# NeSC-IV/sage-icp

Hardware: AMD Instinct MI355X
Metric: ICP frames/sec (120k-pt scan vs 1M-pt map) (higher is better)
Workload: dtype f64

## Files before the change

sage-icp_amd/csrc/icp_body.h:

```cpp
#pragma once

namespace sageicp {

#ifndef SAGE_LOOP_FLAT_MINW
#define SAGE_LOOP_FLAT_MINW 8
#endif
#ifndef SAGE_SCAN_AHEAD
#define SAGE_SCAN_AHEAD 1
#endif
#ifndef SAGE_ROW_SHIFT_LAYER
#define SAGE_ROW_SHIFT_LAYER 1
#endif
#ifndef SAGE_ROW_SHIFT_MAXW
#define SAGE_ROW_SHIFT_MAXW 4
#endif

struct PairCompact {
    uint4 a, b;
    unsigned ka, oa;
    bool ha, hb;
};
struct PairFull {
    Point4 a, b;
    unsigned ka;
// ... 9 lines not shown
    unsigned ka, kb;
    bool ha, hb;
};

__device__ __forceinline__ unsigned icp_wave_of_stripe(const IcpParams &P, int wv, unsigned &stripe_id) {
    constexpr unsigned kStripe = SAGE_ICP_STRIPE;
    const unsigned xcd = blockIdx.x & 7u, jb = blockIdx.x >> 3;
    unsigned stripe = (jb / kStripe) * 8u + xcd;
    if (P.stripe_order) {
        const unsigned nstripes = gridDim.x / kStripe;
        switch (stripe * 4u / nstripes) {
            case 0: __builtin_amdgcn_s_setprio(3); break;
            case 1: __builtin_amdgcn_s_setprio(2); break;
            case 2: __builtin_amdgcn_s_setprio(1); break;
            default: break;
        }
        stripe = P.stripe_order[stripe];
    }
    stripe_id = stripe;
    const unsigned wg = stripe * kStripe + (jb % kStripe);
    return wg * static_cast<unsigned>(kIcpWavesPerBlock) + static_cast<unsigned>(wv);
}

__device__ __forceinline__ void axis_gaps(double v, int k, double vs, double sc, double (&g)[3]) {
    const double below_hi = static_cast<double>(k <= 0 ? k - 1 : k) * vs;
    const double above_lo = static_cast<double>(k >= 0 ? k + 1 : k) * vs;
    const double slack = 1e-9 * vs + 1e-13 * fabs(v);
    const double lo = fmax((v - below_hi) - slack, 0.0);
    const double hi = fmax((above_lo - v) - slack, 0.0);
    g[0] = (lo * lo) * sc;
    g[1] = 0.0;
    g[2] = (hi * hi) * sc;
}

__device__ __forceinline__ float round_up_f32(double x) {
    return __uint_as_float(__float_as_uint(static_cast<float>(x)) + 1u);
}

template <int LW>
__device__ __forceinline__ bool reduce_argmin(double best, unsigned bkey, bool valid, const uint32_t *lrow, unsigned &mkey, unsigned &woff) {
    constexpr int W = 1 << LW, SH = 5;
    const double m = seg_min_f64<W>(best);
    const unsigned mine = (best == m) ? bkey : 0xFFFFFFFFu;
    mkey = seg_min_u32<W>(mine);
    const bool found = valid && mkey != 0xFFFFFFFFu;
    woff = (lrow[found ? mkey >> 8 : 0u] >> 8) * (kUnitPoints * 32u) + ((mkey & 255u) << SH);
    return found;
}

template <int LW, bool FUSED, bool FILT, bool PERSIST = false, bool FLATQ = false>
// ... 76 lines not shown
        f = P.frame[qc];
        auto row_piece = [&](int k) {
            const unsigned p = min(ci + static_cast<unsigned>(W * k), 6u);
            return *reinterpret_cast<const uint4 *>(grow + 4u * p);
        };
        pc0 = row_piece(0); pc1 = pc0; pc2 = pc0; pc3 = pc0; pc4 = pc0; pc5 = pc0; pc6 = pc0;
        if (NP > 1) pc1 = row_piece(1);
        if (NP > 2) pc2 = row_piece(2);
        if (NP > 3) pc3 = row_piece(3);
        if (NP > 4) pc4 = row_piece(4);
        if (NP > 5) pc5 = row_piece(5);
        if (NP > 6) pc6 = row_piece(6);
    }
    PROBE_DELAY_WAIT(P, t0);
    if constexpr (FUSED && !PERSIST) {
        if (P.chain && P.chain_iter > 0) {
            if (wv == 0) chain_wait_pose(P, smem, lane);
            __syncthreads();
            if (smem[kWgGo]) return;
        }
    }
    const Query s = [&]() {
        if constexpr (PERSIST) {
            return make_query<(W >= 4)>(f, pose, pose + 9, 1, P.voxel_size, P.inv_voxel_size);
        } else if constexpr (FUSED) {
            const double *lpose = reinterpret_cast<const double *>(smem + kWgPose);
            return make_query<(W >= 4)>(f, lpose, lpose + 9, P.apply_pose, P.voxel_size, P.inv_voxel_size);
        } else {
            return make_query<(W >= 4)>(f, P.st->R, P.st->T + 4, P.apply_pose, P.voxel_size, P.inv_voxel_size);
        }
    }();
    const bool stale = valid && (static_cast<uint32_t>(s.kx) != rk.x || static_cast<uint32_t>(s.ky) != rk.y ||
                                 static_cast<uint32_t>(s.kz) != rk.z);
    unsigned occ = rk.w;
    NN_T(np, 0);
    LP_T(PERSIST, G, 0);
    if constexpr (!PERSIST) {
        auto stage = [&](int k, const uint4 &v) {
            const unsigned p = ci + static_cast<unsigned>(W * k);
            if (p < 7u) *reinterpret_cast<uint4 *>(lrow + 4u * p) = v;
        };
        stage(0, pc0);
        if (NP > 1) stage(1, pc1);
        if (NP > 2) stage(2, pc2);
        if (NP > 3) stage(3, pc3);
        if (NP > 4) stage(4, pc4);
        if (NP > 5) stage(5, pc5);
        if (NP > 6) stage(6, pc6);
    }
    if (__ballot(stale)) {
        if (stale) {
            unsigned o = 0u, cq = 0u;
// ... 123 lines not shown
                    start(v2, s2, e2);
                    finish(v0, s0, e0);
                    finish(v1, s1, e1);
                    finish(v2, s2, e2);
                }
            }
            o = seg_or_u32<W>(o);
            cq = seg_add_u32<W>(cq);
            occ = o;
            if (ci == 0u) {
                lrow[kRowCq] = cq;
                if constexpr (!PERSIST) {
                    uint4 t;
                    t.x = static_cast<uint32_t>(s.kx); t.y = static_cast<uint32_t>(s.ky);
                    t.z = static_cast<uint32_t>(s.kz); t.w = o;
                    *reinterpret_cast<uint4 *>(P.rows + static_cast<size_t>(q) * kRowWords + kRowKey) = t;
                    P.rows[static_cast<size_t>(q) * kRowWords + kRowCq] = cq;
                }
            }
            if constexpr (PERSIST) {
                if (ci == 0u) {
                    *reinterpret_cast<uint2 *>(lst + kStKey) = make_uint2(static_cast<uint32_t>(s.kx), static_cast<uint32_t>(s.ky));
                    *reinterpret_cast<uint2 *>(lst + kStKey + 2) = make_uint2(static_cast<uint32_t>(s.kz), o);
                }
            }
        }
    }
    if (!valid) occ = 0u;

    double gx[3], gy[3], gz[3];
    {
        const double vs = P.voxel_size, sc = P.prune_scale;
        axis_gaps(s.x, s.kx, vs, sc, gx);
        axis_gaps(s.y, s.ky, vs, sc, gy);
        axis_gaps(s.z, s.kz, vs, sc, gz);
    }
    NN_T(np, 1);
    LP_T(PERSIST, G, 1);

    double best = P.dist_init;
    unsigned bkey = 0xFFFFFFFFu;
    const int pli = static_cast<int>(s.l);
    const double th = P.sem_th;
    unsigned npairs = 0u;

    unsigned k = ci, kend = 0u, off = 0u;
    unsigned pk = 0u, needs = 0u, wn = 0u;
    auto evaluate = [&](const Point4 &nb, bool on, unsigned key) {
        const double dx = nb.x - s.x, dy = nb.y - s.y, dz = nb.z - s.z;
        double d = SAGE_SQNORM3_NN(dx * dx, dy * dy, dz * dz);
        const bool same = static_cast<int>(nb.l) == pli || fabs(nb.l * s.l) < 1.0;
        const double ds = d * th;
        d = same ? ds : d;
        d = __hiloint2double(on ? __double2hiint(d) : 0x7FF80000, __double2loint(d));
        const bool lt = d < best, eq = d == best, kl = key < bkey;
        const bool take = lt | (eq & kl);
        best = min_f64(best, d);
        bkey = take ? key : bkey;
// ... 213 lines not shown
            for (int c = 0; c < 3; ++c) {
                const double lb = ga + (gy[b] + gz[c]);
                layer |= (lb <= bound) ? (1u << (3 * b + c)) : 0u;
            }
        }
        layer = (a < 3u && ci < 4u) ? layer << (9u * a) : 0u;
        layer |= dpp_u32<kDppXor1>(layer);
        layer |= dpp_u32<kDppXor2>(layer);
        if (W >= 8) layer |= dpp_u32<kDppHalfMirror>(layer);
        if (W >= 16) layer |= dpp_u32<kDppMirror>(layer);
        need |= layer & ~(1u << kHome);
    } else {
#pragma unroll
        for (int v = 0; v < 27; ++v) {
            if (v == static_cast<int>(kHome)) continue;
            const double lb = gx[v / 9] + (gy[(v / 3) % 3] + gz[v % 3]);
            need |= (lb <= bound) ? (1u << v) : 0u;
        }
    }
    LP_T(PERSIST, G, 3);
    scan((merged ? (need | (1u << kHome)) : (need & ~(1u << kHome))) & occ, nullptr, false, 0u);
    LP_T(PERSIST, G, 4);
    if constexpr (PERSIST) {
        if (valid && ci == 0u)
            (void)__hip_atomic_fetch_max(G->work + bslot, npairs + (stale ? 48u : 0u), __ATOMIC_RELAXED, __HIP_MEMORY_SCOPE_WORKGROUP);
    }

    unsigned mkey, woff;
    const bool found = reduce_argmin<LW>(best, bkey, valid, lrow, mkey, woff);
    NN_T(np, 3);
    LP_T(PERSIST, G, 5);

    if (P.counters) {
        const unsigned long long ab = (valid && ci == 0u)
                                          ? (static_cast<unsigned long long>(lrow[kRowCq]) << 32) | npairs : 0ull;
        unsigned lo = static_cast<unsigned>(ab), hi = static_cast<unsigned>(ab >> 32);
        lo += dpp_u32<kDppXor1>(lo);        hi += dpp_u32<kDppXor1>(hi);
        lo += dpp_u32<kDppXor2>(lo);        hi += dpp_u32<kDppXor2>(hi);
        lo += dpp_u32<kDppHalfMirror>(lo);  hi += dpp_u32<kDppHalfMirror>(hi);
        lo += dpp_u32<kDppMirror>(lo);      hi += dpp_u32<kDppMirror>(hi);
        unsigned b = 0u, a = 0u;
#pragma unroll
        for (int r = 0; r < 4; ++r) {
            b += static_cast<unsigned>(__builtin_amdgcn_readlane(static_cast<int>(lo), 16 * r));
            a += static_cast<unsigned>(__builtin_amdgcn_readlane(static_cast<int>(hi), 16 * r));
        }
        if (lane == 0 && wave_id < P.nwaves) {
            (void)__hip_atomic_fetch_add(&P.counters[2u * wave_id], static_cast<unsigned long long>(a),
                                         __ATOMIC_RELAXED, __HIP_MEMORY_SCOPE_AGENT);
            (void)__hip_atomic_fetch_add(&P.counters[2u * wave_id + 1u], static_cast<unsigned long long>(b),
                                         __ATOMIC_RELAXED, __HIP_MEMORY_SCOPE_AGENT);
        }
    }

    if (!FUSED) {
        if (valid && ci == 0u) P.nn_idx[q] = found ? static_cast<int>(woff >> SH) : -1;
    } else {
        if constexpr (!PERSIST) {
            if (valid && ci == 0u) P.nn_prev[q] = make_uint2(found ? mkey : 0xFFFFFFFFu, woff);
        }
        Point4 g;
        if constexpr (PERSIST) {
            const bool changed = found && mkey != prev.x;
            g = *reinterpret_cast<const Point4 *>(lst + 8);
            if (__ballot(changed)) {
                const Point4 t = load_point(pts, changed ? woff : 0u);
                if (changed) {
                    g = t;
                    if (ci == 0u) *reinterpret_cast<Point4 *>(lst + 8) = t;
                }
            }
            if (ci == 0u) *reinterpret_cast<uint2 *>(lst + kStPrev) = make_uint2(found ? mkey : 0xFFFFFFFFu, woff);
            LP_T(PERSIST, G, 6);
        }
        PROBE_NN_WORK(P, q, valid && ci == 0u, npairs);
        constexpr int K = kCount >> LW;
        double t[K];
        if constexpr (!PERSIST) g = load_point(pts, found ? woff : 0u);
        const double rx0 = s.x - g.x, ry0 = s.y - g.y, rz0 = s.z - g.z;
        const bool use = found && SAGE_SQNORM3_ACCEPT(rx0 * rx0, ry0 * ry0, rz0 * rz0) <= P.accept_r2;
        {
            const double r2 = SAGE_SQNORM3_RESID(rx0 * rx0, ry0 * ry0, rz0 * rz0);
            const double k = P.kernel;
            const double den = k + r2;
            const double wq = (k * k) / (den * den);
            const bool z = W == 1;
            const double w = !z || use ? wq : 0.0;
            const double sx = !z || use ? s.x : 0.0, sy = !z || use ? s.y : 0.0, sz = !z || use ? s.z : 0.0;
            const double rx = !z || use ? rx0 : 0.0, ry = !z || use ? ry0 : 0.0, rz = !z || use ? rz0 : 0.0;
            const double wsx = w * sx, wsy = w * sy, wsz = w * sz;
            double u[kCount];
            u[kW] = w;
            u[kWsx] = wsx; u[kWsy] = wsy; u[kWsz] = wsz;
            u[kWxx] = wsx * sx; u[kWxy] = wsx * sy; u[kWxz] = wsx * sz;
            u[kWyy] = wsy * sy; u[kWyz] = wsy * sz; u[kWzz] = wsz * sz;
            u[kWrx] = w * rx; u[kWry] = w * ry; u[kWrz] = w * rz;
            u[kWcx] = w * (sy * rz - sz * ry);
            u[kWcy] = w * (sz * rx - sx * rz);
            u[kWcz] = w * (sx * ry - sy * rx);
#pragma unroll
            for (int kk = 0; kk < K; ++kk) {
                double v = u[kk];
#pragma unroll
                for (int l = 1; l < W; ++l) v = ci == static_cast<unsigned>(l) ? u[l * K + kk] : v;
                t[kk] = z || use ? v : 0.0;
            }
        }
        const unsigned pairs = static_cast<unsigned>(__popcll(__ballot(use && ci == 0u)));
        if constexpr (PERSIST) {
            wave_terms_to_wgacc<LW>(t, pairs, lane, G->red, G->wgacc, kDigitLimitCounted, P.acc_scale);
            PROBE_LOOP_WAVE_STATS(smem, valid, ci, npairs, stale, lane);
            LP_T(PERSIST, G, 7);
            return;
        }
        if (P.stripe_work) {
            unsigned mx = valid ? npairs : 0u;
#pragma unroll
            for (int d = 1; d < 64; d <<= 1) mx = max(mx, static_cast<unsigned>(__shfl_xor(mx, d, 64)));
            if (lane == 0) (void)__hip_atomic_fetch_max(&P.stripe_work[stripe_id], mx, __ATOMIC_RELAXED, __HIP_MEMORY_SCOPE_AGENT);
        }
        {
            unsigned long long *wgacc = reinterpret_cast<unsigned long long *>(smem + kWgAcc);
            wave_terms_to_wgacc<LW>(t, pairs, lane, reinterpret_cast<double *>(wl), wgacc, P.digit_limit, P.acc_scale);
            unsigned prior = 0u;
            __atomic_signal_fence(__ATOMIC_SEQ_CST);
            if (lane == 0)
                prior = __hip_atomic_fetch_add(&smem[kWgArrive], 1u, __ATOMIC_RELAXED, __HIP_MEMORY_SCOPE_WORKGROUP);
            __atomic_signal_fence(__ATOMIC_SEQ_CST);
            prior = __builtin_amdgcn_readfirstlane(prior);
            if (prior == kIcpWavesPerBlock - 1u) {
                if (P.chain)
                    wgacc_flush<true>(wgacc, &P.chain->acc32[P.chain_iter & 1][blockIdx.x & (kChainReplicas - 1)][0], nullptr);
                else
// ... 10 lines not shown
```

sage-icp_amd/csrc/kernels.h:

```cpp
#pragma once

#include <hip/hip_runtime.h>

#include "sageicp_types.h"

namespace sageicp {

constexpr int kRowWords = 32;
constexpr int kRowCq = 27, kRowKey = 28, kRowOcc = 31;
constexpr int kRowLdsStride = 36;

struct LoopShared;
struct IcpParams {
    const Point4 *frame;
    int n;
    const IcpState *st;
    int check_done;
    int apply_pose;
    double voxel_size;
    double inv_voxel_size;
    uint32_t *rows;
    const Slot *table;
    uint32_t mask;
    const Point4 *pts;
// ... 87 lines not shown
    LoopShared *sh;
    IcpState *st;
    int nw;
    int gpw;
    int wgs;
    int contiguous;
    uint32_t xcd_first[9];
    unsigned long long timeout_ticks;
    unsigned long long count_timeout_ticks;
    int max_iterations;
    unsigned long long epoch;
    double T0[7];
    double acc_unscale;
    int shared_loop;
    int prio;
    int deal;
    int copies;
    int pose_map;
    IcpProgress *progress;
};
struct LoopArgs {
    IcpParams P;
    LoopParams L;
};
#ifndef SAGE_LOOP_OCC
#define SAGE_LOOP_OCC 7
#endif
constexpr int kLoopMaxWavesHost = 8;
constexpr int kLoopStripeHost = 4;
constexpr int kLoopStateWords = 24;
size_t loop_lds_bytes(int lw, int nw, int gpw);
int loop_blocks_per_cu(int lw, bool filter, int nw, size_t lds);
void launch_loop(const IcpParams &p, const LoopParams &l, int lw, hipStream_t s);
void launch_loop_solve(const LoopParams &l, const P2pParams &x, hipStream_t s);

constexpr int kMaxPartials = 1 << 16;
constexpr uint64_t kMaxQueries = (1ull << 26) - 4;

void launch_tf(Point4 *pts, int n, const IcpState *st, hipStream_t s);
void launch_scatter_points(const uint32_t *idx, const Point4 *vals, uint32_t n, Point4 *pts,
                           hipStream_t s);
void launch_scatter_slots(const uint32_t *idx, const Slot *vals, uint32_t n, Slot *table,
                          hipStream_t s);
void launch_scatter_u32(const uint32_t *idx, const uint32_t *vals, uint32_t n, uint32_t *dst, hipStream_t s);
void launch_sum_counters(const unsigned long long *c, int n, IcpState *st, hipStream_t s);

// ... 82 lines not shown
```

sage-icp_amd/csrc/kernels.hip:

```cpp

#include <hip/hip_runtime.h>

#include <algorithm>
#include <cfloat>
#include <cstdlib>
#include <type_traits>
#include <vector>

#ifndef SAGE_ICP_STRIPE
#define SAGE_ICP_STRIPE 8
#endif
#ifndef SAGE_ICP_OCC
#define SAGE_ICP_OCC 6
#endif

#include "kernels.h"
#include "se3_math.h"
#include "sageicp_types.h"
#include "probes.h"

namespace sageicp {


template <int CTRL>
// ... 136 lines not shown
__device__ __forceinline__ uint32_t probe_voxel(const Slot *table, uint32_t mask, int vx, int vy,
                                                int vz) {
    const uint32_t sl = voxel_hash(vx, vy, vz) & mask;
    const int4 e = reinterpret_cast<const int4 *>(table)[sl];
    return probe_resolve(table, mask, sl, e, vx, vy, vz);
}

struct Query {
    double x, y, z, l;
    int kx, ky, kz;
};
__device__ __forceinline__ int voxel_index(double x, double voxel_size, double inv_vs) {
    const double q = x * inv_vs;
    const bool unsure = !(fabs(q - __builtin_rint(q)) > 1e-9 * (1.0 + fabs(q))) || inv_vs == 0.0;
    int k = static_cast<int>(q);
    if (__ballot(unsure)) {
        asm volatile("" ::: "memory");
        k = static_cast<int>(x / voxel_size);
    }
    return k;
}
template <bool QUAD = false>
__device__ __forceinline__ Query make_query(const Point4 &f, const double *R, const double *t, int apply_pose,
                                            double voxel_size, double inv_vs = 0.0) {
    Query q;
    q.x = f.x; q.y = f.y; q.z = f.z; q.l = f.l;
    if (apply_pose) {
        q.x = R[0] * f.x + R[1] * f.y + R[2] * f.z + t[0];
        q.y = R[3] * f.x + R[4] * f.y + R[5] * f.z + t[1];
        q.z = R[6] * f.x + R[7] * f.y + R[8] * f.z + t[2];
    }
    if constexpr (QUAD) {
        const unsigned a = threadIdx.x & 3u;
        const double num = a == 0u ? q.x : (a == 1u ? q.y : q.z);
        const unsigned k = static_cast<unsigned>(voxel_index(num, voxel_size, inv_vs));
        q.kx = static_cast<int>(dpp_u32<0x00>(k));
        q.ky = static_cast<int>(dpp_u32<0x55>(k));
        q.kz = static_cast<int>(dpp_u32<0xAA>(k));
    } else {
        q.kx = voxel_index(q.x, voxel_size, inv_vs);
        q.ky = voxel_index(q.y, voxel_size, inv_vs);
        q.kz = voxel_index(q.z, voxel_size, inv_vs);
    }
    return q;
}

__global__ __launch_bounds__(256) void k_rows(IcpParams P) {
    const int lane = static_cast<int>(threadIdx.x & 63u);
    const unsigned v = threadIdx.x & 31u;
    const unsigned q = blockIdx.x * 8u + (threadIdx.x >> 5);
    const bool valid = q < static_cast<unsigned>(P.n);
    const Point4 f = P.frame[valid ? q : 0u];
    const Query s = make_query(f, P.st->R, P.st->T + 4, P.apply_pose, P.voxel_size);
    uint32_t w = kEmptySlot;
    if (valid && v < 27u)
        w = probe_voxel(P.table, P.mask, s.kx + static_cast<int>(v / 9u) - 1,
// ... 27 lines not shown
    const double a = __builtin_rint(v);
    const double r1 = (v - a) * 1099511627776.0;
    const double b = __builtin_rint(r1);
    const double c2 = __builtin_rint((r1 - b) * 1099511627776.0);
    ok &= fabs(a) < limit;
    d0 = __double_as_longlong(a + 6755399441055744.0) - 0x4338000000000000ll;
    d1 = __double_as_longlong(b + 6755399441055744.0) - 0x4338000000000000ll;
    d2 = __double_as_longlong(c2 + 6755399441055744.0) - 0x4338000000000000ll;
}
constexpr double kDigitLimitCounted = 1099511627776.0;

template <int CTRL>
__device__ __forceinline__ long long dpp_i64(long long v) {
    int lo = static_cast<int>(v), hi = static_cast<int>(v >> 32);
    lo = __builtin_amdgcn_update_dpp(0, lo, CTRL, 0xF, 0xF, true);
    hi = __builtin_amdgcn_update_dpp(0, hi, CTRL, 0xF, 0xF, true);
    return (static_cast<long long>(hi) << 32) | static_cast<unsigned>(lo);
}
template <int N>
__device__ __forceinline__ double lane_shl_f64(double v) {
    if constexpr (N < 16) return dpp_f64<0x100 + N>(v);
    else return __shfl_down(v, N, 64);
}

template <int LW>
__device__ __forceinline__ void wave_terms_to_wgacc(const double (&t)[kCount >> LW], unsigned pairs, int lane, double *red,
                                                    unsigned long long *wgacc, double limit, double scale) {
    constexpr int W = 1 << LW, QW = 64 >> LW, NBLK = QW / 4, K = kCount >> LW;
    double y[K];
#pragma unroll
    for (int k = 0; k < K; ++k) {
        const double x = t[k] + lane_shl_f64<W>(t[k]);
        y[k] = x + lane_shl_f64<2 * W>(x);
    }
    const int c = lane >> 2, j = lane & 3;
    long long d0 = 0, d1 = 0, d2 = 0;
    bool ok = true;
    const int blk = lane / (4 * W);
    const bool first = (lane & (4 * W - 1)) < W;
#pragma unroll
    for (int r = 0; r < NBLK; r += 4) {
        if (first && blk >= r && blk < r + 4) {
            double *dst = red + (blk - r) * kCount + (lane & (W - 1)) * K;
#pragma unroll
            for (int k = 0; k < K; ++k) dst[k] = y[k];
        }
        __builtin_amdgcn_fence(__ATOMIC_ACQ_REL, "wavefront");
        const double v = r + j < NBLK ? red[j * kCount + c] : 0.0;
        long long e0, e1, e2;
        to_digits(v * scale, limit, e0, e1, e2, ok);
        d0 += e0; d1 += e1; d2 += e2;
        __builtin_amdgcn_fence(__ATOMIC_ACQ_REL, "wavefront");
    }
    (void)__hip_atomic_fetch_add(wgacc + 3 * c, static_cast<unsigned long long>(d0), __ATOMIC_RELAXED, __HIP_MEMORY_SCOPE_WORKGROUP);
    (void)__hip_atomic_fetch_add(wgacc + 3 * c + 1, static_cast<unsigned long long>(d1), __ATOMIC_RELAXED, __HIP_MEMORY_SCOPE_WORKGROUP);
    (void)__hip_atomic_fetch_add(wgacc + 3 * c + 2, static_cast<unsigned long long>(d2), __ATOMIC_RELAXED, __HIP_MEMORY_SCOPE_WORKGROUP);
    if (!ok) (void)__hip_atomic_fetch_or(wgacc + kWgAccWords - 1, 1ull, __ATOMIC_RELAXED, __HIP_MEMORY_SCOPE_WORKGROUP);
    if (lane == 0)
        (void)__hip_atomic_fetch_add(wgacc + 3 * kCount, static_cast<unsigned long long>(pairs), __ATOMIC_RELAXED, __HIP_MEMORY_SCOPE_WORKGROUP);
}

template <bool COUNTED = false>
__device__ __forceinline__ void wgacc_flush(unsigned long long *wgacc, long long *dst, long long *overflow) {
    const int lane = static_cast<int>(threadIdx.x & 63u);
    const int l = min(lane, static_cast<int>(kWgAccWords) - 1);
    const long long x = static_cast<long long>(wgacc[l]);
    const bool ok = wgacc[kWgAccWords - 1] == 0ull;
    __builtin_amdgcn_fence(__ATOMIC_ACQ_REL, "wavefront");
    if (lane < static_cast<int>(kWgAccWords)) wgacc[lane] = 0ull;
    if constexpr (COUNTED) {
        (void)overflow;
        if (lane <= 3 * kAccValues)
            (void)__hip_atomic_fetch_add(dst + lane, lane == 3 * kAccValues ? (ok ? 1ll : 257ll) : (ok ? x * 256 + 1 : 1ll),
                                         __ATOMIC_RELAXED, __HIP_MEMORY_SCOPE_AGENT);
    } else if (lane < 3 * kAccValues) {
        {
            if (ok) (void)__hip_atomic_fetch_add(dst + lane, x, __ATOMIC_RELAXED, __HIP_MEMORY_SCOPE_AGENT);
            else (void)__hip_atomic_fetch_or(overflow, 1ll, __ATOMIC_RELAXED, __HIP_MEMORY_SCOPE_AGENT);
        }
    }
}

struct LoopGroup {
    uint32_t *rows;
    uint32_t *state;
    const uint32_t *perm;
    uint32_t *work;
    unsigned unit;
    double *red;
    unsigned long long *wgacc;
    unsigned q_first;
    unsigned slot;
// ... 3 lines not shown
constexpr unsigned kLoopStripe = kLoopStripeHost;
constexpr int kNoVoxel = 0x7FFFFFFF;
constexpr unsigned kStPrev = 16, kStKey = 18;
constexpr unsigned kLpArrive = 0, kLpNext = 1, kLpDone = 2;
constexpr unsigned kLpPose = 4;
constexpr unsigned kLpDbg = kLpPose + 24u;
constexpr unsigned kLpFirst = kLpDbg + 4u;
constexpr unsigned kLpAcc = kLpFirst + 8u;
constexpr unsigned kLpHeaderWords = (kLpAcc + 2u * kWgAccWords + 15u) & ~15u;
__host__ __device__ constexpr unsigned loop_red_words() { return 2u * kCount * 4u; }
__host__ __device__ constexpr unsigned loop_perm_words(unsigned nblk) { return 2u * ((nblk + 7u) & ~7u); }
template <typename W>
struct LoopLds {
    W perm, work, rows, state, red, end;
    __host__ __device__ constexpr LoopLds(int lw, W nw, W gpw)
        : perm(kLpHeaderWords),
          work(perm + loop_perm_words(static_cast<unsigned>(gpw) * ((64u >> lw) / 4u)) / 2u),
          rows(perm + loop_perm_words(static_cast<unsigned>(gpw) * ((64u >> lw) / 4u))),
          state(rows + gpw * static_cast<W>(64 >> lw) * static_cast<W>(kRowLdsStride)),
          red(state + gpw * static_cast<W>(64 >> lw) * static_cast<W>(kLoopStateWords)),
          end(red + nw * loop_red_words()) {}
};

__device__ __forceinline__ unsigned loop_pose_copy(int pose_map) {
    const unsigned b = blockIdx.x;
    return pose_map == 1 ? 0u : ((pose_map == 2 ? b + 3u : b) & static_cast<unsigned>(kLoopPoseCopies - 1));
}
__device__ __forceinline__ void chain_wait_pose(const IcpParams &P, uint32_t *smem, int lane) {
    LoopShared *sh = P.chain;
    const unsigned long long tag = static_cast<unsigned long long>(P.chain_iter);
    const unsigned long long *src = lane < kLoopPoseGranules ? &sh->pose[loop_pose_copy(P.chain_pose_map)][lane] : &sh->abort_word[0];
    const unsigned long long t0 = __builtin_amdgcn_s_memrealtime();
    unsigned go = 0u;
    unsigned long long g;
    for (;;) {
        g = ld_agent(src);
        const unsigned long long g24 = static_cast<unsigned long long>(static_cast<unsigned>(__builtin_amdgcn_readlane(static_cast<int>(g), 24))) |
                                       (static_cast<unsigned long long>(static_cast<unsigned>(__builtin_amdgcn_readlane(static_cast<int>(g >> 32), 24))) << 32);
        const bool ok = lane >= kLoopPoseGranules || (g >> 32) == tag;
        if (__all(ok)) {
            if (static_cast<uint32_t>(g24) != 0u) go = 1u;
            break;
        }
        if ((g24 >> 32) < tag && static_cast<uint32_t>(g24) != 0u) {
            go = 1u;
            break;
        }
        const bool late = __builtin_amdgcn_s_memrealtime() - t0 > P.chain_timeout;
// ... 226 lines not shown
    switch (lw) {
        case 1: return filter ? SAGE_LOOP_K(1, true) : SAGE_LOOP_K(1, false);
        case 2: return filter ? SAGE_LOOP_K(2, true) : SAGE_LOOP_K(2, false);
        case 3: return filter ? SAGE_LOOP_K(3, true) : SAGE_LOOP_K(3, false);
        case 4: return filter ? SAGE_LOOP_K(4, true) : SAGE_LOOP_K(4, false);
        default: return nullptr;
    }
#undef SAGE_LOOP_K
}
int loop_blocks_per_cu(int lw, bool filter, int nw, size_t lds) {
    if (nw < 1 || nw > kLoopMaxWaves || lds > 160 * 1024) return 0;
    const void *k = loop_kernel(lw, filter);
    if (!k) return 0;
    if (lds > 64 * 1024 && hipFuncSetAttribute(k, hipFuncAttributeMaxDynamicSharedMemorySize, 160 * 1024) != hipSuccess) return 0;
    int nb = 0;
    if (hipOccupancyMaxActiveBlocksPerMultiprocessor(&nb, k, 64 * nw, lds) != hipSuccess) return 0;
    return nb;
}
void launch_loop(const IcpParams &p, const LoopParams &l, int lw, hipStream_t s) {
    const size_t lds = loop_lds_bytes(lw, l.nw, l.gpw);
    LoopArgs a;
    a.P = p;
    a.L = l;
    void *args[] = {&a};
#ifdef SAGE_LOOP_INGRID
    (void)hipLaunchKernel(loop_kernel(lw, p.filter != 0), dim3(l.wgs + 1), dim3(64 * l.nw), args, lds, s);
#else
    (void)hipLaunchKernel(loop_kernel(lw, p.filter != 0), dim3(l.wgs), dim3(64 * l.nw), args, lds, s);
#endif
}
void launch_loop_solve(const LoopParams &l, const P2pParams &x, hipStream_t s) {
    SolveArgs a;
    a.L = l;
    a.X = x;
    if (l.copies == kChainReplicas) hipLaunchKernelGGL(k_loop_solve<kChainReplicas>, dim3(1), dim3(64), 0, s, a);
    else hipLaunchKernelGGL(k_loop_solve<kLoopReplicas>, dim3(1), dim3(64), 0, s, a);
}

int launch_gn(const GnParams &p, hipStream_t s) {
    long blocks = (static_cast<long>(p.n) + 255) / 256;
    if (blocks > 128) blocks = 128;
    if (blocks < 1) blocks = 1;
    hipLaunchKernelGGL(k_gn, dim3(static_cast<int>(blocks)), dim3(256), 0, s, p);
    return static_cast<int>(blocks);
}

// ... 11 lines not shown
```

sage-icp_amd/csrc/loop_kernel.h:

```cpp
#pragma once

namespace sageicp {


__device__ __forceinline__ int exchange_sums_wave(double *S, const P2pParams &X, unsigned long long g) {
    const int lane = static_cast<int>(threadIdx.x & 63u);
    const int slot = static_cast<int>(g & 1ull);
    const unsigned long long tag = g + 1ull;
    if (lane < kNumSums) {
        const double v = S[lane];
        for (int r = 0; r < X.nranks; ++r)
            __hip_atomic_store(&X.block[r]->sums[slot][X.rank][lane], v, __ATOMIC_RELAXED, __HIP_MEMORY_SCOPE_SYSTEM);
    }
    asm volatile("s_waitcnt vmcnt(0)" ::: "memory");
    __builtin_amdgcn_fence(__ATOMIC_RELEASE, "");
    asm volatile("s_waitcnt vmcnt(0)" ::: "memory");
    if (lane == 0)
        for (int r = 0; r < X.nranks; ++r)
            __hip_atomic_store(&X.block[r]->flag[X.rank], tag, __ATOMIC_RELAXED, __HIP_MEMORY_SCOPE_SYSTEM);
    P2pBlock *mine = X.block[X.rank];
    bool late = false, gone = false;
    if (lane < X.nranks) {
        const unsigned long long t0 = __builtin_amdgcn_s_memrealtime();
        while (__hip_atomic_load(&mine->flag[lane], __ATOMIC_RELAXED, __HIP_MEMORY_SCOPE_SYSTEM) < tag) {
// ... 20 lines not shown
}
__device__ __forceinline__ void exchange_abort_wave(const P2pParams &X, unsigned long long g) {
    const int lane = static_cast<int>(threadIdx.x & 63u);
    if (lane == 0)
        for (int r = 0; r < X.nranks; ++r)
            __hip_atomic_store(&X.block[r]->abort_tag[X.rank], g + 1ull, __ATOMIC_RELAXED, __HIP_MEMORY_SCOPE_SYSTEM);
    asm volatile("s_waitcnt vmcnt(0)" ::: "memory");
    __builtin_amdgcn_fence(__ATOMIC_RELEASE, "");
    asm volatile("s_waitcnt vmcnt(0)" ::: "memory");
    if (lane == 0)
        for (int r = 0; r < X.nranks; ++r)
            __hip_atomic_store(&X.block[r]->flag[X.rank], g + 1ull, __ATOMIC_RELAXED, __HIP_MEMORY_SCOPE_SYSTEM);
    asm volatile("s_waitcnt vmcnt(0)" ::: "memory");
}

struct SolveLds {
    double T[14];
    double S[kNumSums];
};
__device__ __forceinline__ unsigned long long readlane_u64(unsigned long long v, int src) {
    const unsigned lo = static_cast<unsigned>(__builtin_amdgcn_readlane(static_cast<int>(static_cast<unsigned>(v)), src));
    const unsigned hi = static_cast<unsigned>(__builtin_amdgcn_readlane(static_cast<int>(static_cast<unsigned>(v >> 32)), src));
    return (static_cast<unsigned long long>(hi) << 32) | lo;
}
__device__ __forceinline__ int lane_now() {
    unsigned l;
    asm volatile("v_mbcnt_lo_u32_b32 %0, -1, 0\n\tv_mbcnt_hi_u32_b32 %0, -1, %0" : "=v"(l));
    return static_cast<int>(l);
}
__device__ __forceinline__ void loop_give_up(const LoopParams &L, LoopShared *sh, IcpState *st, int it, unsigned long long tag, int lane,
                                             bool peer) {
    if (lane == 0) {
        st_agent(&sh->abort_word[0], 1ull);
        st->loop_aborted = 1;
        if (peer) st->peer_aborted = 1;
        if (L.progress)
            __hip_atomic_store(&L.progress->word, (1ull << 32) | static_cast<unsigned long long>(it), __ATOMIC_RELAXED,
                               __HIP_MEMORY_SCOPE_SYSTEM);
    }
    if (const int al = lane_now(); al < kLoopPoseCopies) st_agent(&sh->pose[al][24], (tag << 32) | 2ull);
}
template <int COPIES>
__device__ __forceinline__ unsigned loop_finish_iteration(const LoopParams &L, const P2pParams &X, SolveLds &m, int it,
                                                          unsigned long long &xg) {
    LoopShared *sh = L.sh;
    IcpState *st = L.st;
    const int lane = static_cast<int>(threadIdx.x & 63u);
    double *sT = m.T, *S = m.S;
    const unsigned long long tag = static_cast<unsigned long long>(it) + 1ull;

    double sum = 0.0;
// ... 217 lines not shown
        for (int it = 0;; ++it)
            if (loop_finish_iteration<kLoopReplicas>(L, X, m, it, xg)) return;
    }
#endif

    unsigned g0, gcnt;
    {
        const unsigned xcd = blockIdx.x & 7u, jb = blockIdx.x >> 3;
        const unsigned ngroups = (static_cast<unsigned>(P.n) + QW - 1u) / QW;
        unsigned lo = 0u, cnt = ngroups, idx, nwg;
        if (L.contiguous == 1) {
            lo = L.xcd_first[xcd];
            cnt = L.xcd_first[xcd + 1u] - lo;
            idx = jb;
            nwg = static_cast<unsigned>(L.wgs) >> 3;
        } else {
            idx = ((jb / kLoopStripe) * 8u + xcd) * kLoopStripe + (jb % kLoopStripe);
            nwg = static_cast<unsigned>(L.wgs);
        }
        const unsigned base = cnt / nwg, extra = cnt - base * nwg;
        g0 = lo + idx * base + min(idx, extra);
        gcnt = min(gpw, base + (idx < extra ? 1u : 0u));
    }
    unsigned long long *wgacc = reinterpret_cast<unsigned long long *>(smem + kLpAcc);
    constexpr unsigned BPW = QW / 4;
    const unsigned nblk_max = gpw * BPW, nblk = gcnt * BPW;
    const LoopLds<unsigned> lds(LW, static_cast<unsigned>(nw), gpw);
    uint32_t *perm = smem + lds.perm;
    uint32_t *work = smem + lds.work;
    uint32_t *rows = smem + lds.rows;
    uint32_t *state = smem + lds.state;
    double *red = reinterpret_cast<double *>(smem + lds.red + static_cast<unsigned>(wv) * loop_red_words());

    if (threadIdx.x < 9) s_pose[threadIdx.x] = P.st->R[threadIdx.x];
    else if (threadIdx.x < 12) s_pose[threadIdx.x] = P.st->T[4 + threadIdx.x - 9];
    if (threadIdx.x == 0) {
        smem[kLpArrive] = 0u;
        smem[kLpNext] = 0u;
        smem[kLpDone] = 0u;
        PROBE_LOOP_CLEAR_STATS(smem);
    }
    if (L.deal && (threadIdx.x & 63u) == 0u) {
        unsigned hw;
        asm volatile("s_getreg_b32 %0, hwreg(HW_REG_HW_ID)" : "=s"(hw));
        smem[kLpFirst + static_cast<unsigned>(wv)] = (((hw >> 4) & 3u) + (hw & 15u)) % static_cast<unsigned>(nw);
    }
    for (unsigned i = threadIdx.x; i < 2u * kWgAccWords; i += blockDim.x) smem[kLpAcc + i] = 0u;
    for (unsigned i = threadIdx.x; i < nblk_max; i += blockDim.x) {
        perm[i] = i;
        work[i] = 0u;
    }
    for (unsigned sl = threadIdx.x; sl < gcnt * QW; sl += blockDim.x) {
        const unsigned q = g0 * QW + sl;
        const Point4 f = P.frame[q < static_cast<unsigned>(P.n) ? q : 0u];
        {
            uint32_t *lst = state + sl * kLoopStateWords;
            *reinterpret_cast<Point4 *>(lst) = f;
            Point4 z;
            z.x = z.y = z.z = z.l = 0.0;
            *reinterpret_cast<Point4 *>(lst + 8) = z;
            *reinterpret_cast<uint4 *>(lst + kStPrev) = make_uint4(0xFFFFFFFFu, 0u, static_cast<uint32_t>(kNoVoxel),
                                                                   static_cast<uint32_t>(kNoVoxel));
            *reinterpret_cast<uint4 *>(lst + kStPrev + 4) = make_uint4(static_cast<uint32_t>(kNoVoxel), 0u, 0u, 0u);
        }
    }
    __syncthreads();
    if (L.deal) {
        unsigned claimed = 0u, kept = 0u, table[kLoopMaxWaves];
        for (int w2 = 0; w2 < nw; ++w2) {
            const unsigned pr = smem[kLpFirst + static_cast<unsigned>(w2)];
            table[w2] = pr;
            if (!((claimed >> pr) & 1u)) { claimed |= 1u << pr; kept |= 1u << w2; }
        }
        for (int w2 = 0; w2 < nw; ++w2)
            if (!((kept >> w2) & 1u)) {
                const unsigned pr = static_cast<unsigned>(__builtin_ctz(~claimed));
                table[w2] = pr;
                claimed |= 1u << pr;
            }
        __syncthreads();
        if (threadIdx.x == 0) {
            for (int w2 = 0; w2 < nw; ++w2) smem[kLpFirst + static_cast<unsigned>(w2)] = table[w2];
            smem[kLpNext] = static_cast<unsigned>(nw);
        }
        __syncthreads();
    }
    PROBE_LOOP_BEGIN(lp);

    for (int it = 0;; ++it) {
        auto ka = __builtin_amdgcn_kernarg_segment_ptr();
        asm volatile("" : "+s"(ka));
        const LoopArgs &K = *(const LoopArgs *)(ka);
        const LoopParams &L = K.L;
        LoopShared *sh = L.sh;
        unsigned lane_u;
        asm volatile("v_mbcnt_lo_u32_b32 %0, -1, 0\n\tv_mbcnt_hi_u32_b32 %0, -1, %0" : "=v"(lane_u));
        const int lane = static_cast<int>(lane_u);
        bool dealt = L.deal != 0;
        for (;;) {
            unsigned gi = 0u;
            if (dealt) {
                dealt = false;
                gi = static_cast<unsigned>(__builtin_amdgcn_readfirstlane(static_cast<int>(smem[kLpFirst + static_cast<unsigned>(wv)])));
                if (gi >= gcnt) continue;
            } else {
                if (lane == 0)
                    gi = __hip_atomic_fetch_add(&smem[kLpNext], 1u, __ATOMIC_RELAXED, __HIP_MEMORY_SCOPE_WORKGROUP);
                gi = static_cast<unsigned>(__builtin_amdgcn_readfirstlane(static_cast<int>(gi)));
                if (gi >= gcnt) break;
            }
            if (L.prio) loop_set_priority(gi, nw, L.prio);
            PROBE_LOOP_UNIT_BEGIN(it, gi, nw, t_unit);
            LoopGroup G;
            G.rows = rows;
            G.state = state;
            G.perm = perm;
            G.work = work;
            G.unit = gi;
            G.red = red;
            G.wgacc = wgacc;
            G.q_first = g0 * QW;
            G.slot = g0 + gi;
            PROBE_LOOP_PASS_BEGIN(lp, G);
            {
                auto kb = __builtin_amdgcn_kernarg_segment_ptr();
                asm volatile("" : "+s"(kb));
                icp_body<LW, true, FILT, true>(((const LoopArgs *)(kb))->P, smem, &G, s_pose);
            }
            PROBE_LOOP_UNIT_END(lp, G, it, gi, nw, wv, lane, t_unit);
        }
        PROBE_LOOP_MARK(t_a);
        unsigned prior = 0u;
        __atomic_signal_fence(__ATOMIC_SEQ_CST);
        if (lane == 0)
            prior = __hip_atomic_fetch_add(&smem[kLpArrive], 1u, __ATOMIC_RELAXED, __HIP_MEMORY_SCOPE_WORKGROUP);
        __atomic_signal_fence(__ATOMIC_SEQ_CST);
        prior = static_cast<unsigned>(__builtin_amdgcn_readfirstlane(static_cast<int>(prior)));
        const bool last = prior == static_cast<unsigned>(nw) - 1u;
        if (last) {
            wgacc_flush<true>(wgacc, &sh->acc[it & 1][blockIdx.x & (kLoopReplicas - 1)][0], &sh->acc[it & 1][0][kAccWords - 1]);
            if (lane == 0) {
                smem[kLpArrive] = 0u;
                smem[kLpNext] = L.deal ? static_cast<unsigned>(nw) : 0u;
            }
            if (nblk <= 64u && nblk > BPW) {
                __builtin_amdgcn_fence(__ATOMIC_ACQ_REL, "wavefront");
                const unsigned i = static_cast<unsigned>(lane);
                const unsigned wi = i < nblk ? work[i] : 0u;
                unsigned rank = 0u;
                for (unsigned j = 0; j < nblk; ++j) {
                    const unsigned wj = work[j];
                    rank += (wj > wi || (wj == wi && j < i)) ? 1u : 0u;
                }
                __builtin_amdgcn_fence(__ATOMIC_ACQ_REL, "wavefront");
                if (i < nblk) {
                    perm[rank] = i;
                    work[i] = 0u;
                }
            }
            PROBE_LOOP_WG_INFO(smem, it, lane);
            LOOP_STAMP_WG(it, 0);
        }
        if (wv == 0) {
            const unsigned long long tag = static_cast<unsigned long long>(it) + 1ull;
            const unsigned long long t0 = __builtin_amdgcn_s_memrealtime();
            unsigned long long g = tag << 32;
            bool aborted = false;
            for (;;) {
                if (lane < kLoopPoseGranules) g = ld_agent(&sh->pose[loop_pose_copy(L.pose_map)][lane]);
                const bool ok = (g >> 32) == tag;
                if (__all(ok)) break;
                unsigned long long ab = 0ull;
                if (lane == 0) ab = ld_agent(&sh->abort_word[0]);
                const bool late = __builtin_amdgcn_s_memrealtime() - t0 > L.timeout_ticks;
                if (__any(ab != 0ull) || late) {
                    if (lane == 0 && late) {
                        st_agent(&sh->abort_word[0], 1ull);
                        L.st->loop_aborted = 1;
                    }
                    aborted = true;
                    break;
                }
                __builtin_amdgcn_s_sleep(SAGE_LOOP_POLL_SLEEP);
                if (L.wgs > 1024) __builtin_amdgcn_s_sleep(SAGE_LOOP_POLL_SLEEP);
            }
            if (aborted) {
                if (lane == 0) smem[kLpDone] = 2u;
            } else {
                if (lane < 24) reinterpret_cast<uint32_t *>(s_pose)[lane] = static_cast<uint32_t>(g);
                if (lane == 24) smem[kLpDone] = static_cast<uint32_t>(g);
            }
            LOOP_STAMP_WG(it, 1);
// ... 11 lines not shown
```

Measured before the change: 237.4.

## Rematerialize loop-invariant values in persistent loop to cut register pressure

Recomputes LDS pointers, lane index, wave/block IDs and kernel arguments at their point of use inside the persistent ICP loop instead of keeping them live across the body. It packs the block and wave index into one opaque scalar and recomputes the lane with mbcnt. It also reloads the state pointer and previous key from LDS after the scan, and moves the face slack into a kernel argument. The goal is fewer live VGPRs/SGPRs across the heavy icp_body call, which should mean fewer spills or higher occupancy. The cost is extra recomputation and LDS reads, and the deep-shift reduction now uses ds_bpermute instead of shfl.

```diff
diff --git a/sage-icp_amd/csrc/icp_body.h b/sage-icp_amd/csrc/icp_body.h
--- a/sage-icp_amd/csrc/icp_body.h
+++ b/sage-icp_amd/csrc/icp_body.h
@@ -55,10 +55,11 @@
     return wg * static_cast<unsigned>(kIcpWavesPerBlock) + static_cast<unsigned>(wv);
 }
 
-__device__ __forceinline__ void axis_gaps(double v, int k, double vs, double sc, double (&g)[3]) {
+template <bool GIVEN>
+__device__ __forceinline__ void axis_gaps(double v, int k, double vs, double sc, double fs, double (&g)[3]) {
     const double below_hi = static_cast<double>(k <= 0 ? k - 1 : k) * vs;
     const double above_lo = static_cast<double>(k >= 0 ? k + 1 : k) * vs;
-    const double slack = 1e-9 * vs + 1e-13 * fabs(v);
+    const double slack = (GIVEN ? fs : 1e-9 * vs) + 1e-13 * fabs(v);
     const double lo = fmax((v - below_hi) - slack, 0.0);
     const double hi = fmax((above_lo - v) - slack, 0.0);
     g[0] = (lo * lo) * sc;
@@ -181,12 +182,12 @@
     }
     const Query s = [&]() {
         if constexpr (PERSIST) {
-            return make_query<(W >= 4)>(f, pose, pose + 9, 1, P.voxel_size, P.inv_voxel_size);
+            return make_query<(W >= 4)>(f, pose, pose + 9, 1, P.voxel_size, P.inv_voxel_size, static_cast<unsigned>(lane));
         } else if constexpr (FUSED) {
             const double *lpose = reinterpret_cast<const double *>(smem + kWgPose);
-            return make_query<(W >= 4)>(f, lpose, lpose + 9, P.apply_pose, P.voxel_size, P.inv_voxel_size);
+            return make_query<(W >= 4)>(f, lpose, lpose + 9, P.apply_pose, P.voxel_size, P.inv_voxel_size, threadIdx.x);
         } else {
-            return make_query<(W >= 4)>(f, P.st->R, P.st->T + 4, P.apply_pose, P.voxel_size, P.inv_voxel_size);
+            return make_query<(W >= 4)>(f, P.st->R, P.st->T + 4, P.apply_pose, P.voxel_size, P.inv_voxel_size, threadIdx.x);
         }
     }();
     const bool stale = valid && (static_cast<uint32_t>(s.kx) != rk.x || static_cast<uint32_t>(s.ky) != rk.y ||
@@ -356,18 +357,25 @@
                 if (ci == 0u) {
                     *reinterpret_cast<uint2 *>(lst + kStKey) = make_uint2(static_cast<uint32_t>(s.kx), static_cast<uint32_t>(s.ky));
                     *reinterpret_cast<uint2 *>(lst + kStKey + 2) = make_uint2(static_cast<uint32_t>(s.kz), o);
-                }
-            }
-        }
+                    lst[kStPrev] = prev.x;
+                }
+            }
+        }
+    }
+    if constexpr (PERSIST) {
+        __builtin_amdgcn_fence(__ATOMIC_ACQ_REL, "wavefront");
+        prev.x = lst[opaque_v(kStPrev)];
     }
     if (!valid) occ = 0u;
 
     double gx[3], gy[3], gz[3];
     {
         const double vs = P.voxel_size, sc = P.prune_scale;
-        axis_gaps(s.x, s.kx, vs, sc, gx);
-        axis_gaps(s.y, s.ky, vs, sc, gy);
-        axis_gaps(s.z, s.kz, vs, sc, gz);
+        double fs = 0.0;
+        if constexpr (PERSIST) fs = reinterpret_cast<const LoopArgs *>(&P)->face_slack;
+        axis_gaps<PERSIST>(s.x, s.kx, vs, sc, fs, gx);
+        axis_gaps<PERSIST>(s.y, s.ky, vs, sc, fs, gy);
+        axis_gaps<PERSIST>(s.z, s.kz, vs, sc, fs, gz);
     }
     NN_T(np, 1);
     LP_T(PERSIST, G, 1);
@@ -627,8 +635,12 @@
     scan((merged ? (need | (1u << kHome)) : (need & ~(1u << kHome))) & occ, nullptr, false, 0u);
     LP_T(PERSIST, G, 4);
     if constexpr (PERSIST) {
+        lane = lane_now();
+        const unsigned qe = static_cast<unsigned>(lane) >> LW;
+        const unsigned bs = G->perm[G->unit * (QW / 4) + (qe >> 2)];
+        lst = G->state + (bs * 4u + (qe & 3u)) * kLoopStateWords;
         if (valid && ci == 0u)
-            (void)__hip_atomic_fetch_max(G->work + bslot, npairs + (stale ? 48u : 0u), __ATOMIC_RELAXED, __HIP_MEMORY_SCOPE_WORKGROUP);
+            (void)__hip_atomic_fetch_max(G->work + bs, npairs + (stale ? 48u : 0u), __ATOMIC_RELAXED, __HIP_MEMORY_SCOPE_WORKGROUP);
     }
 
     unsigned mkey, woff;
@@ -666,7 +678,7 @@
         }
         Point4 g;
         if constexpr (PERSIST) {
-            const bool changed = found && mkey != prev.x;
+            const bool changed = found && mkey != lst[opaque_v(kStPrev)];
             g = *reinterpret_cast<const Point4 *>(lst + 8);
             if (__ballot(changed)) {
                 const Point4 t = load_point(pts, changed ? woff : 0u);
@@ -713,7 +725,7 @@
         }
         const unsigned pairs = static_cast<unsigned>(__popcll(__ballot(use && ci == 0u)));
         if constexpr (PERSIST) {
-            wave_terms_to_wgacc<LW>(t, pairs, lane, G->red, G->wgacc, kDigitLimitCounted, P.acc_scale);
+            wave_terms_to_wgacc<LW, true>(t, pairs, lane, G->red, G->wgacc, kDigitLimitCounted, P.acc_scale);
             PROBE_LOOP_WAVE_STATS(smem, valid, ci, npairs, stale, lane);
             LP_T(PERSIST, G, 7);
             return;
diff --git a/sage-icp_amd/csrc/kernels.h b/sage-icp_amd/csrc/kernels.h
--- a/sage-icp_amd/csrc/kernels.h
+++ b/sage-icp_amd/csrc/kernels.h
@@ -133,6 +133,7 @@
 struct LoopArgs {
     IcpParams P;
     LoopParams L;
+    double face_slack;
 };
 #ifndef SAGE_LOOP_OCC
 #define SAGE_LOOP_OCC 7
diff --git a/sage-icp_amd/csrc/kernels.hip b/sage-icp_amd/csrc/kernels.hip
--- a/sage-icp_amd/csrc/kernels.hip
+++ b/sage-icp_amd/csrc/kernels.hip
@@ -182,7 +182,7 @@
 }
 template <bool QUAD = false>
 __device__ __forceinline__ Query make_query(const Point4 &f, const double *R, const double *t, int apply_pose,
-                                            double voxel_size, double inv_vs = 0.0) {
+                                            double voxel_size, double inv_vs = 0.0, unsigned quad_lane = 0u) {
     Query q;
     q.x = f.x; q.y = f.y; q.z = f.z; q.l = f.l;
     if (apply_pose) {
@@ -191,7 +191,7 @@
         q.z = R[6] * f.x + R[7] * f.y + R[8] * f.z + t[2];
     }
     if constexpr (QUAD) {
-        const unsigned a = threadIdx.x & 3u;
+        const unsigned a = quad_lane & 3u;
         const double num = a == 0u ? q.x : (a == 1u ? q.y : q.z);
         const unsigned k = static_cast<unsigned>(voxel_index(num, voxel_size, inv_vs));
         q.kx = static_cast<int>(dpp_u32<0x00>(k));
@@ -265,16 +265,31 @@
     if constexpr (N < 16) return dpp_f64<0x100 + N>(v);
     else return __shfl_down(v, N, 64);
 }
-
-template <int LW>
+template <int N>
+__device__ __forceinline__ double lane_shl_f64_at(double v, int lane) {
+    if constexpr (N < 16) {
+        return dpp_f64<0x100 + N>(v);
+    } else {
+        const int a = ((lane + N) & 63) << 2;
+        const int lo = __builtin_amdgcn_ds_bpermute(a, __double2loint(v)), hi = __builtin_amdgcn_ds_bpermute(a, __double2hiint(v));
+        return __hiloint2double(hi, lo);
+    }
+}
+
+template <int LW, bool FRESH = false>
 __device__ __forceinline__ void wave_terms_to_wgacc(const double (&t)[kCount >> LW], unsigned pairs, int lane, double *red,
                                                     unsigned long long *wgacc, double limit, double scale) {
     constexpr int W = 1 << LW, QW = 64 >> LW, NBLK = QW / 4, K = kCount >> LW;
     double y[K];
 #pragma unroll
     for (int k = 0; k < K; ++k) {
-        const double x = t[k] + lane_shl_f64<W>(t[k]);
-        y[k] = x + lane_shl_f64<2 * W>(x);
+        if constexpr (FRESH) {
+            const double x = t[k] + lane_shl_f64_at<W>(t[k], lane);
+            y[k] = x + lane_shl_f64_at<2 * W>(x, lane);
+        } else {
+            const double x = t[k] + lane_shl_f64<W>(t[k]);
+            y[k] = x + lane_shl_f64<2 * W>(x);
+        }
     }
     const int c = lane >> 2, j = lane & 3;
     long long d0 = 0, d1 = 0, d2 = 0;
@@ -303,14 +318,35 @@
         (void)__hip_atomic_fetch_add(wgacc + 3 * kCount, static_cast<unsigned long long>(pairs), __ATOMIC_RELAXED, __HIP_MEMORY_SCOPE_WORKGROUP);
 }
 
-template <bool COUNTED = false>
+__device__ __forceinline__ int lane_now() {
+    unsigned l;
+    asm volatile("v_mbcnt_lo_u32_b32 %0, -1, 0\n\tv_mbcnt_hi_u32_b32 %0, -1, %0" : "=v"(l));
+    return static_cast<int>(l);
+}
+__device__ __forceinline__ unsigned opaque_s(unsigned x) {
+    asm volatile("" : "+s"(x));
+    return x;
+}
+
+__device__ __forceinline__ unsigned opaque_v(unsigned x) {
+    asm volatile("" : "+v"(x));
+    return x;
+}
+
+template <bool COUNTED = false, bool FRESH = false>
 __device__ __forceinline__ void wgacc_flush(unsigned long long *wgacc, long long *dst, long long *overflow) {
-    const int lane = static_cast<int>(threadIdx.x & 63u);
+    const int lane = FRESH ? lane_now() : static_cast<int>(threadIdx.x & 63u);
     const int l = min(lane, static_cast<int>(kWgAccWords) - 1);
     const long long x = static_cast<long long>(wgacc[l]);
     const bool ok = wgacc[kWgAccWords - 1] == 0ull;
     __builtin_amdgcn_fence(__ATOMIC_ACQ_REL, "wavefront");
-    if (lane < static_cast<int>(kWgAccWords)) wgacc[lane] = 0ull;
+    unsigned long long zero = 0ull;
+    if constexpr (FRESH) {
+        unsigned zl, zh;
+        asm volatile("v_mov_b32 %0, 0\n\tv_mov_b32 %1, 0" : "=v"(zl), "=v"(zh));
+        zero = (static_cast<unsigned long long>(zh) << 32) | zl;
+    }
+    if (lane < static_cast<int>(kWgAccWords)) wgacc[lane] = zero;
     if constexpr (COUNTED) {
         (void)overflow;
         if (lane <= 3 * kAccValues)
@@ -360,8 +396,7 @@
           end(red + nw * loop_red_words()) {}
 };
 
-__device__ __forceinline__ unsigned loop_pose_copy(int pose_map) {
-    const unsigned b = blockIdx.x;
+__device__ __forceinline__ unsigned loop_pose_copy(int pose_map, unsigned b = blockIdx.x) {
     return pose_map == 1 ? 0u : ((pose_map == 2 ? b + 3u : b) & static_cast<unsigned>(kLoopPoseCopies - 1));
 }
 __device__ __forceinline__ void chain_wait_pose(const IcpParams &P, uint32_t *smem, int lane) {
@@ -634,6 +669,7 @@
     LoopArgs a;
     a.P = p;
     a.L = l;
+    a.face_slack = 1e-9 * p.voxel_size;
     void *args[] = {&a};
 #ifdef SAGE_LOOP_INGRID
     (void)hipLaunchKernel(loop_kernel(lw, p.filter != 0), dim3(l.wgs + 1), dim3(64 * l.nw), args, lds, s);
diff --git a/sage-icp_amd/csrc/loop_kernel.h b/sage-icp_amd/csrc/loop_kernel.h
--- a/sage-icp_amd/csrc/loop_kernel.h
+++ b/sage-icp_amd/csrc/loop_kernel.h
@@ -66,11 +66,6 @@
     const unsigned lo = static_cast<unsigned>(__builtin_amdgcn_readlane(static_cast<int>(static_cast<unsigned>(v)), src));
     const unsigned hi = static_cast<unsigned>(__builtin_amdgcn_readlane(static_cast<int>(static_cast<unsigned>(v >> 32)), src));
     return (static_cast<unsigned long long>(hi) << 32) | lo;
-}
-__device__ __forceinline__ int lane_now() {
-    unsigned l;
-    asm volatile("v_mbcnt_lo_u32_b32 %0, -1, 0\n\tv_mbcnt_hi_u32_b32 %0, -1, %0" : "=v"(l));
-    return static_cast<int>(l);
 }
 __device__ __forceinline__ void loop_give_up(const LoopParams &L, LoopShared *sh, IcpState *st, int it, unsigned long long tag, int lane,
                                              bool peer) {
@@ -334,15 +329,12 @@
         g0 = lo + idx * base + min(idx, extra);
         gcnt = min(gpw, base + (idx < extra ? 1u : 0u));
     }
-    unsigned long long *wgacc = reinterpret_cast<unsigned long long *>(smem + kLpAcc);
     constexpr unsigned BPW = QW / 4;
-    const unsigned nblk_max = gpw * BPW, nblk = gcnt * BPW;
-    const LoopLds<unsigned> lds(LW, static_cast<unsigned>(nw), gpw);
-    uint32_t *perm = smem + lds.perm;
-    uint32_t *work = smem + lds.work;
-    uint32_t *rows = smem + lds.rows;
-    uint32_t *state = smem + lds.state;
-    double *red = reinterpret_cast<double *>(smem + lds.red + static_cast<unsigned>(wv) * loop_red_words());
+    const unsigned nblk_max = gpw * BPW;
+    const LoopLds<unsigned> lds0(LW, static_cast<unsigned>(nw), gpw);
+    uint32_t *perm0 = smem + lds0.perm;
+    uint32_t *work0 = smem + lds0.work;
+    uint32_t *state0 = smem + lds0.state;
 
     if (threadIdx.x < 9) s_pose[threadIdx.x] = P.st->R[threadIdx.x];
     else if (threadIdx.x < 12) s_pose[threadIdx.x] = P.st->T[4 + threadIdx.x - 9];
@@ -359,14 +351,14 @@
     }
     for (unsigned i = threadIdx.x; i < 2u * kWgAccWords; i += blockDim.x) smem[kLpAcc + i] = 0u;
     for (unsigned i = threadIdx.x; i < nblk_max; i += blockDim.x) {
-        perm[i] = i;
-        work[i] = 0u;
+        perm0[i] = i;
+        work0[i] = 0u;
     }
     for (unsigned sl = threadIdx.x; sl < gcnt * QW; sl += blockDim.x) {
         const unsigned q = g0 * QW + sl;
         const Point4 f = P.frame[q < static_cast<unsigned>(P.n) ? q : 0u];
         {
-            uint32_t *lst = state + sl * kLoopStateWords;
+            uint32_t *lst = state0 + sl * kLoopStateWords;
             *reinterpret_cast<Point4 *>(lst) = f;
             Point4 z;
             z.x = z.y = z.z = z.l = 0.0;
@@ -397,65 +389,73 @@
         }
         __syncthreads();
     }
+    static_assert(kLoopMaxWaves <= 8, "k_loop keeps the wave's index in three bits");
+    const unsigned who = (blockIdx.x << 3) | static_cast<unsigned>(wv);
     PROBE_LOOP_BEGIN(lp);
+
 
     for (int it = 0;; ++it) {
         auto ka = __builtin_amdgcn_kernarg_segment_ptr();
         asm volatile("" : "+s"(ka));
-        const LoopArgs &K = *(const LoopArgs *)(ka);
-        const LoopParams &L = K.L;
-        LoopShared *sh = L.sh;
-        unsigned lane_u;
-        asm volatile("v_mbcnt_lo_u32_b32 %0, -1, 0\n\tv_mbcnt_hi_u32_b32 %0, -1, %0" : "=v"(lane_u));
-        const int lane = static_cast<int>(lane_u);
-        bool dealt = L.deal != 0;
+        bool dealt = ((const LoopArgs *)(ka))->L.deal != 0;
         for (;;) {
             unsigned gi = 0u;
             if (dealt) {
                 dealt = false;
-                gi = static_cast<unsigned>(__builtin_amdgcn_readfirstlane(static_cast<int>(smem[kLpFirst + static_cast<unsigned>(wv)])));
-                if (gi >= gcnt) continue;
+                gi = static_cast<unsigned>(__builtin_amdgcn_readfirstlane(static_cast<int>(smem[kLpFirst + (opaque_s(who) & 7u)])));
+                if (gi >= opaque_s(gcnt)) continue;
             } else {
-                if (lane == 0)
+                if (lane_now() == 0)
                     gi = __hip_atomic_fetch_add(&smem[kLpNext], 1u, __ATOMIC_RELAXED, __HIP_MEMORY_SCOPE_WORKGROUP);
                 gi = static_cast<unsigned>(__builtin_amdgcn_readfirstlane(static_cast<int>(gi)));
-                if (gi >= gcnt) break;
-            }
-            if (L.prio) loop_set_priority(gi, nw, L.prio);
-            PROBE_LOOP_UNIT_BEGIN(it, gi, nw, t_unit);
+                if (gi >= opaque_s(gcnt)) break;
+            }
+            auto kb = __builtin_amdgcn_kernarg_segment_ptr();
+            asm volatile("" : "+s"(kb));
+            const LoopArgs &B = *(const LoopArgs *)(kb);
+            if (B.L.prio) loop_set_priority(gi, B.L.nw, B.L.prio);
+            PROBE_LOOP_UNIT_BEGIN(it, gi, B.L.nw, t_unit);
+            const LoopLds<unsigned> lds(LW, static_cast<unsigned>(B.L.nw), static_cast<unsigned>(B.L.gpw));
+            const unsigned first = opaque_s(g0);
             LoopGroup G;
-            G.rows = rows;
-            G.state = state;
-            G.perm = perm;
-            G.work = work;
+            G.rows = smem + lds.rows;
+            G.state = smem + lds.state;
+            G.perm = smem + lds.perm;
+            G.work = smem + lds.work;
             G.unit = gi;
-            G.red = red;
-            G.wgacc = wgacc;
-            G.q_first = g0 * QW;
-            G.slot = g0 + gi;
+            G.red = reinterpret_cast<double *>(smem + lds.red + (opaque_s(who) & 7u) * loop_red_words());
+            G.wgacc = reinterpret_cast<unsigned long long *>(smem + kLpAcc);
+            G.q_first = first * QW;
+            G.slot = first + gi;
             PROBE_LOOP_PASS_BEGIN(lp, G);
-            {
-                auto kb = __builtin_amdgcn_kernarg_segment_ptr();
-                asm volatile("" : "+s"(kb));
-                icp_body<LW, true, FILT, true>(((const LoopArgs *)(kb))->P, smem, &G, s_pose);
-            }
-            PROBE_LOOP_UNIT_END(lp, G, it, gi, nw, wv, lane, t_unit);
+            icp_body<LW, true, FILT, true>(B.P, smem, &G, s_pose);
+            PROBE_LOOP_UNIT_END(lp, G, it, gi, B.L.nw, static_cast<int>(opaque_s(who) & 7u), lane_now(), t_unit);
         }
         PROBE_LOOP_MARK(t_a);
+        auto kc = __builtin_amdgcn_kernarg_segment_ptr();
+        asm volatile("" : "+s"(kc));
+        const LoopParams &L = ((const LoopArgs *)(kc))->L;
+        LoopShared *sh = L.sh;
+        const int lane = lane_now();
+        const unsigned me = opaque_s(who), wg = me >> 3;
         unsigned prior = 0u;
         __atomic_signal_fence(__ATOMIC_SEQ_CST);
         if (lane == 0)
             prior = __hip_atomic_fetch_add(&smem[kLpArrive], 1u, __ATOMIC_RELAXED, __HIP_MEMORY_SCOPE_WORKGROUP);
         __atomic_signal_fence(__ATOMIC_SEQ_CST);
         prior = static_cast<unsigned>(__builtin_amdgcn_readfirstlane(static_cast<int>(prior)));
-        const bool last = prior == static_cast<unsigned>(nw) - 1u;
+        const bool last = prior == static_cast<unsigned>(L.nw) - 1u;
         if (last) {
-            wgacc_flush<true>(wgacc, &sh->acc[it & 1][blockIdx.x & (kLoopReplicas - 1)][0], &sh->acc[it & 1][0][kAccWords - 1]);
+            wgacc_flush<true, true>(reinterpret_cast<unsigned long long *>(smem + kLpAcc), &sh->acc[it & 1][wg & (kLoopReplicas - 1)][0],
+                                    &sh->acc[it & 1][0][kAccWords - 1]);
             if (lane == 0) {
                 smem[kLpArrive] = 0u;
-                smem[kLpNext] = L.deal ? static_cast<unsigned>(nw) : 0u;
-            }
+                smem[kLpNext] = L.deal ? static_cast<unsigned>(L.nw) : 0u;
+            }
+            const unsigned nblk = opaque_s(gcnt) * BPW;
             if (nblk <= 64u && nblk > BPW) {
+                const LoopLds<unsigned> lds(LW, static_cast<unsigned>(L.nw), static_cast<unsigned>(L.gpw));
+                uint32_t *perm = smem + lds.perm, *work = smem + lds.work;
                 __builtin_amdgcn_fence(__ATOMIC_ACQ_REL, "wavefront");
                 const unsigned i = static_cast<unsigned>(lane);
                 const unsigned wi = i < nblk ? work[i] : 0u;
@@ -473,13 +473,13 @@
             PROBE_LOOP_WG_INFO(smem, it, lane);
             LOOP_STAMP_WG(it, 0);
         }
-        if (wv == 0) {
+        if ((me & 7u) == 0u) {
             const unsigned long long tag = static_cast<unsigned long long>(it) + 1ull;
             const unsigned long long t0 = __builtin_amdgcn_s_memrealtime();
             unsigned long long g = tag << 32;
             bool aborted = false;
             for (;;) {
-                if (lane < kLoopPoseGranules) g = ld_agent(&sh->pose[loop_pose_copy(L.pose_map)][lane]);
+                if (lane < kLoopPoseGranules) g = ld_agent(&sh->pose[loop_pose_copy(L.pose_map, wg)][lane]);
                 const bool ok = (g >> 32) == tag;
                 if (__all(ok)) break;
                 unsigned long long ab = 0ull;
```

After: 244.9 (median of 6 runs). 3.2% higher.
